# sangminwoo/Temporal-Span-Proposal-Network-VidVRD

Measured on AMD Instinct MI355X. Metric: tracklet-pairs/sec scored (N=32, T=150, D=2048), higher is better.
Workload: dtype f32

## Files before the change

### temporal-span-proposal-network-vidvrd_amd/csrc/tspn_wino63.hip

```cpp
#include <algorithm>
#include <atomic>
#include <type_traits>

#include "tspn_common.h"
#include "tspn_device.h"

namespace {

using namespace tspn_dev;

constexpr int NW = 4;
constexpr int THREADS = 64 * NW;
constexpr int BM = 128;
constexpr int ST = 32;
constexpr int SWG = 64;
constexpr int KC = 8;
constexpr int NJ = 8;
constexpr int VROW = ST * 4;
constexpr int VCH = 2 * NJ * VROW;
constexpr int VHALF = 4 * VCH;
constexpr int VSS = 2 * VHALF;
constexpr int NVB = 2;
constexpr int NPIECE = 16;
constexpr size_t SMEM_BYTES = sizeof(float) * NVB * VSS;
#ifndef TSPN_WINO63_GM
#define TSPN_WINO63_GM 4
#endif

#ifndef TSPN_WINO63_VAUX
#define TSPN_WINO63_VAUX 0
#endif

__global__ void pack_wino63_frag_kernel(const float* __restrict__ W, int64_t M, int64_t Cin, int64_t split,
                                        float* __restrict__ out) {
  const int64_t Mp = split ? 2 * M : M, Cp = split ? split : Cin;
  const int64_t nch = Cp / KC;
  const int64_t total = NJ * Cp * Mp;
  for (int64_t o = blockIdx.x * (int64_t)blockDim.x + threadIdx.x; o < total;
       o += (int64_t)gridDim.x * blockDim.x) {
    const int e = (int)(o & 3);
    const int lane = (int)((o >> 2) & 63);
    const int64_t r = o >> 8;
    const int j = (int)(r % NJ);
    const int64_t c = (r / NJ) % nch;
    const int64_t mb = r / (NJ * nch);
    const int64_t ch = 8 * c + 4 * (lane >> 5) + e;
    const int64_t m = 32 * mb + (lane & 31);
    const float* g = (split && m >= M) ? W + ((m - M) * Cin + split + ch) * 3 : W + (m * Cin + ch) * 3;
    const double g0 = g[0], g1 = g[1], g2 = g[2];
    double u;
    switch (j) {
      case 0: u = g0; break;
      case 1: u = -2.0 / 9.0 * (g0 + g1 + g2); break;
      case 2: u = -2.0 / 9.0 * (g0 - g1 + g2); break;
      case 3: u = g0 / 90.0 + g1 / 45.0 + 2.0 * g2 / 45.0; break;
      case 4: u = g0 / 90.0 - g1 / 45.0 + 2.0 * g2 / 45.0; break;
      case 5: u = (32.0 * g0 + 16.0 * g1 + 8.0 * g2) / 45.0; break;
      case 6: u = (32.0 * g0 - 16.0 * g1 + 8.0 * g2) / 45.0; break;
      default: u = g2; break;
    }
    out[o] = (float)u;
  }
}

__device__ __forceinline__ void wino63_load_sextet(const float* __restrict__ x, int64_t b, int q, int T, int Cin,
                                                   int64_t ncols, bool ok, int channel_offset, f32x4 (&d)[8]) {
#pragma unroll
  for (int i = 0; i < 8; ++i) {
    const int t = 6 * q + i - 1;
    int64_t n = b * T + t;
    n = n < 0 ? 0 : (n < ncols ? n : ncols - 1);
    const f32x4 v = *reinterpret_cast<const f32x4*>(x + n * Cin + channel_offset);
    d[i] = (ok && t >= 0 && t < T) ? v : f32x4{0.f, 0.f, 0.f, 0.f};
  }
}
__device__ __forceinline__ void wino63_bt(const f32x4 (&d)[8], f32x4 (&V)[8]) {
  V[0] = d[0] - d[6] + 5.25f * (d[4] - d[2]);
  V[7] = d[7] - d[1] + 5.25f * (d[3] - d[5]);
  {
    const f32x4 t1 = d[2] + d[6] - 4.25f * d[4], t2 = d[1] + d[5] - 4.25f * d[3];
    V[1] = t1 + t2;
    V[2] = t1 - t2;
  }
  {
    const f32x4 t1 = d[6] + 0.25f * d[2] - 1.25f * d[4], t2 = 0.5f * d[1] - 2.5f * d[3] + 2.f * d[5];
    V[3] = t1 + t2;
    V[4] = t1 - t2;
  }
  {
    const f32x4 t1 = d[6] + 4.f * (d[2] - 1.25f * d[4]), t2 = 2.f * d[1] - 2.5f * d[3] + 0.5f * d[5];
    V[5] = t1 + t2;
    V[6] = t1 - t2;
  }
}
__device__ __forceinline__ void wino63_absmax_own_frames(const f32x4 (&d)[8], float& m) {
#pragma unroll
  for (int i = 1; i < 7; ++i)
    m = __builtin_elementwise_maximum(
        __builtin_elementwise_maximum(m, __builtin_elementwise_maximum(fabsf(d[i][0]), fabsf(d[i][1]))),
        __builtin_elementwise_maximum(fabsf(d[i][2]), fabsf(d[i][3])));
}
__device__ __forceinline__ void wino63_hot_publish(unsigned long long* __restrict__ hot, unsigned long long key, unsigned slot) {
  key = tspn::wave_max_u64(key);
  if ((threadIdx.x & 63) == 0)
    __hip_atomic_fetch_max(hot + 32 * (slot & (TSPN_CONV_CHECK_HOT_SLOTS - 1)), key, __ATOMIC_RELAXED,
                           __HIP_MEMORY_SCOPE_AGENT);
}

__global__ __launch_bounds__(256) void wino63_input_transform_kernel(
    const float* __restrict__ x, float* __restrict__ Vg, int T, int Cin, int nq, int64_t nsext, int64_t nsp,
    int64_t ncols, unsigned long long* __restrict__ hot) {
  const int lane = threadIdx.x & 63, wave = threadIdx.x >> 6;
  const int cgl = lane & 7, ql = lane >> 3;
  const int64_t S = ((int64_t)blockIdx.x * 4 + wave) * 8 + ql;
  const int cg = blockIdx.y * 8 + cgl;
  if (4 * cg >= Cin) return;
  const bool ok = S < nsext;
  const int64_t b = ok ? S / nq : 0;
  const int q = ok ? (int)(S - b * nq) : 0;
  f32x4 d[8], V[8];
  wino63_load_sextet(x, b, q, T, Cin, ncols, ok, 4 * cg, d);
  if (hot) {
    float m = 0.f;
    wino63_absmax_own_frames(d, m);
    wino63_hot_publish(hot, ((unsigned long long)__float_as_uint(m) << 32) | (unsigned)(S < nsext ? S : 0),
                       blockIdx.x * 4 + wave + 7 * blockIdx.y);
  }
  wino63_bt(d, V);
#pragma unroll
  for (int j = 0; j < 8; ++j)
    *reinterpret_cast<f32x4*>(Vg + (((int64_t)cg * NJ + j) * nsp + S) * 4) = V[j];
}

template <bool BUFV>
__global__ __launch_bounds__(THREADS) __attribute__((amdgpu_waves_per_eu(1, 1))) void conv3_wino63_kernel(
    const float* __restrict__ Vg, const float* __restrict__ Wf, const float* __restrict__ bias,
    float* __restrict__ y, int Cin, int T, int M, int nq, int64_t nsext, int64_t nsp, int tiles_m,
    int tiles_n, int relu, int ldy, int GM, int vec2) {
  extern __shared__ __attribute__((aligned(16))) char smem_raw[];
  float* Vs = reinterpret_cast<float*>(smem_raw);

  int tile_m, tile_n;
  grouped_tile(xcd_remap(blockIdx.x, gridDim.x), GM, tiles_m, tiles_n, tile_m, tile_n);
  const int m0 = tile_m * BM;
  const int64_t S0 = (int64_t)tile_n * SWG;

  const int tid = threadIdx.x;
  const int lane = tid & 63;
  const int wave = __builtin_amdgcn_readfirstlane(tid >> 6);
  const int li = lane & 31, kh = lane >> 5;
  const int nsuper = Cin >> 5;

  const char* abase;
  const unsigned aoff = lane * 16;
  {
    int mb = (m0 >> 5) + wave;
    mb = mb < (M >> 5) ? mb : 0;
    abase = reinterpret_cast<const char*>(Wf) + (int64_t)mb * (Cin / KC) * (NJ * 64 * 16);
  }

  const float* vsrc[BUFV ? 1 : NPIECE];
  unsigned voff[BUFV ? NPIECE : 1];
#pragma unroll
  for (int k = 0; k < NPIECE; ++k) {
    const int pp = NPIECE * wave + k;
    const int rr = 2 * (pp & 31) + kh;
    const int cl = rr >> 4, rem = rr & 15;
    const int g = rem >> 3, j = rem & 7;
    const int64_t e = (((int64_t)(2 * cl + g) * NJ + j) * nsp + S0 + ST * (pp >> 5) + li) * 4;
    if constexpr (BUFV) voff[k] = (unsigned)(e * 4); else vsrc[k] = Vg + e;
  }
  const int64_t super_step = (int64_t)8 * NJ * nsp * 4;
  const __amdgpu_buffer_rsrc_t rsrc_v = buffer_rsrc(Vg, (int)0xffffffffu);
  const unsigned super_bytes = (unsigned)(super_step * 4);
  auto stage_piece = [&](int S, int k) {
    if constexpr (BUFV) {
      const int soff = (int)((unsigned)S * super_bytes);
      bglds16(rsrc_v, voff[k], soff, Vs + (S & 1) * VSS + (NPIECE * wave + k) * 256);
    } else {
      glds16<TSPN_WINO63_VAUX>(vsrc[k], Vs + (S & 1) * VSS + (NPIECE * wave + k) * 256);
    }
    if constexpr (!BUFV) vsrc[k] += super_step;
  };

  f32x16 acc[2][NJ];
#pragma unroll
  for (int cb = 0; cb < 2; ++cb)
#pragma unroll
    for (int j = 0; j < NJ; ++j)
#pragma unroll
      for (int e = 0; e < 16; ++e) acc[cb][j][e] = 0.f;

  f32x4 a[2][NJ], v[2][NJ];
  const float* vlane = Vs + (kh * NJ * ST + li) * 4;
  auto load_v = [&](const float* vbuf, int cl, int j) {
    v[0][j] = *reinterpret_cast<const f32x4*>(vbuf + cl * VCH + j * VROW);
    v[1][j] = *reinterpret_cast<const f32x4*>(vbuf + VHALF + cl * VCH + j * VROW);
  };
  auto load_a_pair = [&](f32x4* ap, auto jp_tag, const char* base) {
    constexpr int JP = decltype(jp_tag)::value;
    if (JP == 0) { load_wfrag<0>(ap[0], aoff, base); load_wfrag<1024>(ap[1], aoff, base); }
    if (JP == 1) { load_wfrag<2048>(ap[2], aoff, base); load_wfrag<3072>(ap[3], aoff, base); }
    if (JP == 2) { load_wfrag<0>(ap[4], aoff, base + 4096); load_wfrag<1024>(ap[5], aoff, base + 4096); }
    if (JP == 3) { load_wfrag<2048>(ap[6], aoff, base + 4096); load_wfrag<3072>(ap[7], aoff, base + 4096); }
  };
  using P0 = std::integral_constant<int, 0>;
  using P1 = std::integral_constant<int, 1>;
  using P2 = std::integral_constant<int, 2>;
  using P3 = std::integral_constant<int, 3>;
  auto mfma_pair = [&](const f32x4* ap, int ja, int jb, int S1, int slot) {
#pragma unroll
    for (int e = 0; e < 4; ++e) {
      acc[0][ja] = __builtin_amdgcn_mfma_f32_32x32x2f32(ap[ja][e], v[0][ja][e], acc[0][ja], 0, 0, 0);
      acc[0][jb] = __builtin_amdgcn_mfma_f32_32x32x2f32(ap[jb][e], v[0][jb][e], acc[0][jb], 0, 0, 0);
      acc[1][ja] = __builtin_amdgcn_mfma_f32_32x32x2f32(ap[ja][e], v[1][ja][e], acc[1][ja], 0, 0, 0);
      if (S1 >= 0) {
        __builtin_amdgcn_sched_barrier(0);
        stage_piece(S1, 4 * slot + e);
        __builtin_amdgcn_sched_barrier(0);
      }
      acc[1][jb] = __builtin_amdgcn_mfma_f32_32x32x2f32(ap[jb][e], v[1][jb][e], acc[1][jb], 0, 0, 0);
    }
  };

#pragma unroll
  for (int k = 0; k < NPIECE; ++k) stage_piece(0, k);
  asm volatile("s_waitcnt vmcnt(0)" ::: "memory");
  __syncthreads();
#pragma unroll
  for (int j = 0; j < NJ; ++j) load_v(vlane, 0, j);
  load_a_pair(a[0], P0{}, abase); load_a_pair(a[0], P1{}, abase); load_a_pair(a[0], P2{}, abase); load_a_pair(a[0], P3{}, abase);
  abase += NJ * 1024;
  load_a_pair(a[1], P0{}, abase); load_a_pair(a[1], P1{}, abase); load_a_pair(a[1], P2{}, abase); load_a_pair(a[1], P3{}, abase);
  abase += NJ * 1024;
  __builtin_amdgcn_sched_barrier(0);

  auto chunk_body = [&](auto cl_tag, const float* vcur, const float* vnext, int S, auto has1_tag, auto has2_tag,
                        auto more_tag) {
    constexpr int CL = decltype(cl_tag)::value;
    constexpr bool HAS1 = decltype(has1_tag)::value;
    constexpr bool HAS2 = decltype(has2_tag)::value;
    constexpr bool MORE = decltype(more_tag)::value;
    constexpr int PAR = CL & 1;
    constexpr int N1 = (HAS1 ? 8 : 0) + ((MORE && CL == 1) ? NPIECE : 0);
    constexpr int N2 = (MORE && CL == 2) ? 6 : 2;
    constexpr int N0 = (HAS2 ? 2 : 0) + ((MORE && CL == 0) ? 4 : 0);
    const int S1 = (MORE && CL == 0) ? S + 1 : -1;
    const float* vn = CL == 3 ? vnext : vcur;
    constexpr int NCL = (CL + 1) & 3;
    f32x4* ap = a[PAR];
    wait_w<3 * N2 + N1>(ap[0], ap[1]);
    mfma_pair(ap, 0, 1, S1, 0);
    if (HAS2) load_a_pair(ap, P0{}, abase);
    if (HAS1) { load_v(vn, NCL, 0); load_v(vn, NCL, 1); }
    __builtin_amdgcn_sched_barrier(0);
    wait_w<2 * N2 + N1 + N0>(ap[2], ap[3]);
    mfma_pair(ap, 2, 3, S1, 1);
    if (HAS2) load_a_pair(ap, P1{}, abase);
    if (HAS1) { load_v(vn, NCL, 2); load_v(vn, NCL, 3); }
    __builtin_amdgcn_sched_barrier(0);
    wait_w<N2 + N1 + 2 * N0>(ap[4], ap[5]);
    mfma_pair(ap, 4, 5, S1, 2);
    if (HAS2) load_a_pair(ap, P2{}, abase);
    if (HAS1) { load_v(vn, NCL, 4); load_v(vn, NCL, 5); }
    __builtin_amdgcn_sched_barrier(0);
    wait_w<N1 + 3 * N0>(ap[6], ap[7]);
    mfma_pair(ap, 6, 7, S1, 3);
    if (HAS2) {
      load_a_pair(ap, P3{}, abase);
      abase += NJ * 1024;
    }
    if (HAS1) { load_v(vn, NCL, 6); load_v(vn, NCL, 7); }
    __builtin_amdgcn_sched_barrier(0);
    if (MORE && CL == 2) {
      asm volatile("s_waitcnt lgkmcnt(0)" ::: "memory");
      __builtin_amdgcn_s_barrier();
      __builtin_amdgcn_sched_barrier(0);
    }
  };
  {
    using TT = std::true_type;
    using FF = std::false_type;
    using C0 = std::integral_constant<int, 0>;
    using C1 = std::integral_constant<int, 1>;
    using C2 = std::integral_constant<int, 2>;
    using C3 = std::integral_constant<int, 3>;
    int S = 0;
    for (; S + 1 < nsuper; ++S) {
      const float* vcur = vlane + (S & 1) * VSS;
      const float* vnext = vlane + ((S + 1) & 1) * VSS;
      chunk_body(C0{}, vcur, vnext, S, TT{}, TT{}, TT{});
      chunk_body(C1{}, vcur, vnext, S, TT{}, TT{}, TT{});
      chunk_body(C2{}, vcur, vnext, S, TT{}, TT{}, TT{});
      chunk_body(C3{}, vcur, vnext, S, TT{}, TT{}, TT{});
    }
    const float* vcur = vlane + (S & 1) * VSS;
    chunk_body(C0{}, vcur, vcur, S, TT{}, TT{}, FF{});
    chunk_body(C1{}, vcur, vcur, S, TT{}, TT{}, FF{});
    chunk_body(C2{}, vcur, vcur, S, TT{}, FF{}, FF{});
    chunk_body(C3{}, vcur, vcur, S, FF{}, FF{}, FF{});
  }

#pragma unroll
  for (int cb = 0; cb < 2; ++cb) {
    const int64_t Sx = S0 + ST * cb + li;
    if (Sx < nsext) {
      const int64_t b = Sx / nq;
      const int q = (int)(Sx - b * nq);
      const int t = 6 * q;
      float* ycol = y + (b * M) * (int64_t)ldy + t;
#pragma unroll
      for (int e = 0; e < 16; ++e) {
        const int m = m0 + wave * 32 + (e & 3) + 8 * (e >> 2) + 4 * kh;
        if (m < M) {
          const float p12 = acc[cb][1][e] + acc[cb][2][e], m12 = acc[cb][1][e] - acc[cb][2][e];
          const float p34 = acc[cb][3][e] + acc[cb][4][e], m34 = acc[cb][3][e] - acc[cb][4][e];
          const float p56 = acc[cb][5][e] + acc[cb][6][e], m56 = acc[cb][5][e] - acc[cb][6][e];
          float o[6];
          o[0] = acc[cb][0][e] + p12 + p34 + p56;
          o[1] = m12 + 2.f * m34 + 0.5f * m56;
          o[2] = p12 + 4.f * p34 + 0.25f * p56;
          o[3] = m12 + 8.f * m34 + 0.125f * m56;
          o[4] = p12 + 16.f * p34 + 0.0625f * p56;
          o[5] = m12 + 32.f * m34 + 0.03125f * m56 + acc[cb][7][e];
          if (bias != nullptr) {
            const float bb = bias[m];
#pragma unroll
            for (int i = 0; i < 6; ++i) o[i] += bb;
          }
          if (relu) {
#pragma unroll
            for (int i = 0; i < 6; ++i) o[i] = tspn::relu_f32(o[i]);
          }
          float* dst = ycol + (int64_t)m * ldy;
          if (vec2) {
            *reinterpret_cast<f32x2*>(dst) = f32x2{o[0], o[1]};
            *reinterpret_cast<f32x2*>(dst + 2) = f32x2{o[2], o[3]};
            *reinterpret_cast<f32x2*>(dst + 4) = f32x2{o[4], o[5]};
          } else {
#pragma unroll
            for (int i = 0; i < 6; ++i)
              if (t + i < T) dst[i] = o[i];
          }
        }
      }
    }
  }
}

constexpr int F_BM = 256, F_BN = 256;
constexpr int F_THREADS = 512;
constexpr int F_ST = 4 * 2 * 256 * 16;
constexpr int F_NST = 4;
constexpr size_t F_SMEM = (size_t)F_NST * F_ST;
constexpr size_t F_SMEM_ALL = F_SMEM + 2 * 256 * sizeof(int);
static_assert(TSPN_WINO63_GM > 0 && TSPN_WINO63_GM < 256, "the contraction's GM argument carries the tail split and the piece form above bit 7");
constexpr size_t F_PARK_PER_TILE = (size_t)7 * F_THREADS * 128 * sizeof(float);

__device__ __forceinline__ int split_exponent(double mx) {
  if (!(mx > 0.0) || !(mx <= 1.7976931348623157e308)) return 0;
  int k;
  (void)frexp(mx, &k);
  return 15 - k;
}

__device__ __forceinline__ double wino63_u(int j, double g0, double g1, double g2) {
  switch (j) {
    case 0: return g0;
    case 1: return -2.0 / 9.0 * (g0 + g1 + g2);
    case 2: return -2.0 / 9.0 * (g0 - g1 + g2);
    case 3: return g0 / 90.0 + g1 / 45.0 + 2.0 * g2 / 45.0;
    case 4: return g0 / 90.0 - g1 / 45.0 + 2.0 * g2 / 45.0;
    case 5: return (32.0 * g0 + 16.0 * g1 + 8.0 * g2) / 45.0;
    case 6: return (32.0 * g0 - 16.0 * g1 + 8.0 * g2) / 45.0;
    default: return g2;
  }
}

__global__ void pack_wino63_frag_kernel(const float* __restrict__ W, int64_t M, int64_t Cin, int64_t split,
                                        int16_t* __restrict__ out) {
  const int64_t Mp = split ? 2 * M : M, Cp = split ? split : Cin;
  const int64_t ncg = Cp / 8;
  const int64_t o = blockIdx.x * (int64_t)blockDim.x + threadIdx.x;
  if (o >= NJ * Mp) return;
  const int j = (int)(o / Mp);
  const int64_t m = o - j * Mp;
  const float* g = (split && m >= M) ? W + ((m - M) * Cin + split) * 3 : W + (m * Cin) * 3;
  double mx = 0.0;
  for (int64_t c = 0; c < Cp; ++c) {
    const double u = fabs(wino63_u(j, g[3 * c], g[3 * c + 1], g[3 * c + 2]));
    mx = (u > mx || u != u) ? u : mx;
  }
  const int e = split_exponent(mx);
  int16_t* pj = out + (int64_t)j * (2 * ncg + 1) * Mp * 8;
  for (int64_t cg = 0; cg < ncg; ++cg) {
    f16x8 hi, lo;
#pragma unroll
    for (int i = 0; i < 8; ++i) {
      const int64_t c = 8 * cg + i;
      const double u = ldexp(wino63_u(j, g[3 * c], g[3 * c + 1], g[3 * c + 2]), e);
      const _Float16 h = (_Float16)(float)u;
      hi[i] = h;
      lo[i] = (_Float16)(float)(u - (double)(float)h);
    }
    *reinterpret_cast<f16x8*>(pj + (cg * Mp + m) * 8) = hi;
    *reinterpret_cast<f16x8*>(pj + ((ncg + cg) * Mp + m) * 8) = lo;
  }
  *reinterpret_cast<int4*>(pj + (2 * ncg * Mp + m) * 8) = int4{e, 0, 0, 0};
}

__global__ __launch_bounds__(256) void wino63_input_transform_kernel(
    const float* __restrict__ x, _Float16* __restrict__ Vh, int* __restrict__ Ve, int T, int Cin, int nq,
    int64_t nsext, int64_t nsp2, int64_t ncols, unsigned long long* __restrict__ hot) {
  __shared__ float red[4][8][NJ];
  const int tid = threadIdx.x, lane = tid & 63, wave = tid >> 6;
  const int s = tid & 7, cgs = tid >> 3;
  const int64_t S = (int64_t)blockIdx.x * 8 + s;
  const bool ok = S < nsext;
  const int64_t b = ok ? S / nq : 0;
  const int q = ok ? (int)(S - b * nq) : 0;
  const int ncg = Cin >> 3;
  auto transform = [&](int cg, f32x4 (&V)[2][8], bool want_max, float& xmax) {
#pragma unroll
    for (int h = 0; h < 2; ++h) {
      f32x4 d[8];
      wino63_load_sextet(x, b, q, T, Cin, ncols, ok, 8 * cg + 4 * h, d);
      if (want_max) wino63_absmax_own_frames(d, xmax);
      wino63_bt(d, V[h]);
    }
  };
  float cmax[NJ];
#pragma unroll
  for (int j = 0; j < NJ; ++j) cmax[j] = 0.f;
  float xm = 0.f;
  for (int cg = cgs; cg < ncg; cg += 32) {
    f32x4 V[2][8];
    transform(cg, V, hot != nullptr, xm);
#pragma unroll
    for (int j = 0; j < NJ; ++j)
#pragma unroll
      for (int h = 0; h < 2; ++h)
        cmax[j] = __builtin_elementwise_maximum(
            __builtin_elementwise_maximum(cmax[j], __builtin_elementwise_maximum(fabsf(V[h][j][0]), fabsf(V[h][j][1]))),
            __builtin_elementwise_maximum(fabsf(V[h][j][2]), fabsf(V[h][j][3])));
  }
  if (hot)
    wino63_hot_publish(hot, ((unsigned long long)__float_as_uint(xm) << 32) | (unsigned)(ok ? S : 0),
                       blockIdx.x * 4 + wave);
#pragma unroll
  for (int j = 0; j < NJ; ++j) {
    float m = cmax[j];
#pragma unroll
    for (int o = 8; o < 64; o <<= 1) m = __builtin_elementwise_maximum(m, __shfl_xor(m, o, 64));
    if (lane < 8) red[wave][lane][j] = m;
  }
  __syncthreads();
  int ecol[NJ];
#pragma unroll
  for (int j = 0; j < NJ; ++j) {
    const float m = __builtin_elementwise_maximum(__builtin_elementwise_maximum(red[0][s][j], red[1][s][j]),
                                                  __builtin_elementwise_maximum(red[2][s][j], red[3][s][j]));
    ecol[j] = split_exponent((double)m);
  }
  if (cgs == 0) {
#pragma unroll
    for (int j = 0; j < NJ; ++j) Ve[(int64_t)j * nsp2 + S] = ecol[j];
  }
  for (int cg = cgs; cg < ncg; cg += 32) {
    f32x4 V[2][8];
    transform(cg, V, false, xm);
#pragma unroll
    for (int j = 0; j < NJ; ++j) {
      f16x8 hi, lo;
#pragma unroll
      for (int i = 0; i < 8; ++i) {
        const float u = ldexpf(V[i >> 2][j][i & 3], ecol[j]);
        const _Float16 h = (_Float16)u;
        hi[i] = h;
        lo[i] = (_Float16)(u - (float)h);
      }
      _Float16* dst = Vh + (((int64_t)j * 2 * ncg + cg) * nsp2 + S) * 8;
      *reinterpret_cast<f16x8*>(dst) = hi;
      *reinterpret_cast<f16x8*>(dst + (int64_t)ncg * nsp2 * 8) = lo;
    }
  }
}

#ifndef TSPN_WINO63_F16X3_STAGGER
#define TSPN_WINO63_F16X3_STAGGER 1
#endif
template <int WN, bool BUF>
__device__ __forceinline__ void wino63_f16x3_tile(
    char* smem_raw, const _Float16* __restrict__ Vh, const int* __restrict__ Ve, const int16_t* __restrict__ Wp,
    const float* __restrict__ bias, float* __restrict__ y, float* __restrict__ park, int Cin, int T, int M, int nq,
    int64_t nsext, int64_t nsp2, int tile_m, int tile_n, int tiles_n, int sub, int relu, int ldy, int vec2) {
  constexpr int MI = WN;
  constexpr int BN = 64 * WN;
  constexpr int NP = 16 + 4 * WN;
  constexpr int PW = (NP + 7) / 8;
  constexpr bool EVEN = NP % 8 == 0;
  constexpr bool STAGGER = TSPN_WINO63_F16X3_STAGGER && WN == 4;
  const int m0 = tile_m * F_BM;
  const int64_t S0 = (int64_t)tile_n * F_BN + sub * BN;

  const int tid = threadIdx.x;
  const int lane = tid & 63;
  const int wave = __builtin_amdgcn_readfirstlane(tid >> 6);
  const int wm = wave / WN, wn = wave % WN;
  const int li = lane & 31, kh = lane >> 5;
  const int ncg = Cin >> 3, nk = Cin >> 4;
  const int G = NJ * nk;

  const int p0 = wave * NP / 8;
  const int npw = EVEN ? PW : (wave + 1) * NP / 8 - p0;
  const int16_t* src[PW];
  unsigned voff[PW];
  int ldst[PW];
#pragma unroll
  for (int i = 0; i < PW; ++i) {
    const int p = min(p0 + i, NP - 1);
    int64_t el;
    if (p < 16) {
      const int region = p >> 3, cgi = (p >> 2) & 1, r = 64 * (p & 3) + lane;
      el = (((int64_t)region * ncg + cgi) * M + m0 + r) * 8;
      src[i] = Wp + el;
      ldst[i] = p * 1024;
    } else {
      const int v = p - 16;
      const int region = v / (2 * WN), cgi = (v / WN) & 1, r = 64 * (v % WN) + lane;
      el = (((int64_t)region * ncg + cgi) * nsp2 + S0 + r) * 8;
      src[i] = reinterpret_cast<const int16_t*>(Vh) + el;
      ldst[i] = (2 + region) * 8192 + cgi * 4096 + (v % WN) * 1024;
    }
    voff[i] = (unsigned)(el * 2);
  }
  int ik = 0, ist = 0;
  const char* wbase = reinterpret_cast<const char*>(Wp);
  const char* vbase = reinterpret_cast<const char*>(Vh);
  auto issue = [&]() {
    char* dst = smem_raw + ist * F_ST;
#pragma unroll
    for (int i = 0; i < PW; ++i)
      if (EVEN || i < npw) {
        if (BUF) bglds16(buffer_rsrc_unbounded(p0 + i < 16 ? wbase : vbase), voff[i], 0, dst + ldst[i]);
        else glds16(src[i], dst + ldst[i]);
      }
    ist = (ist + 1) & 3;
    const bool wrap = ++ik == nk;
    if (wrap) ik = 0;
    const int64_t dw = (int64_t)M * (wrap ? 32 * nk + 48 : 32), dv = nsp2 * (wrap ? 32 * nk + 32 : 32);
    if (BUF) {
      wbase += dw;
      vbase += dv;
    } else {
#pragma unroll
      for (int i = 0; i < PW; ++i) src[i] = reinterpret_cast<const int16_t*>(reinterpret_cast<const char*>(src[i]) + (p0 + i < 16 ? dw : dv));
    }
  };
  auto wait_stages = [&](auto ahead_tag) {
    constexpr int AHEAD = decltype(ahead_tag)::value;
    if (EVEN || npw == PW) wait_vmcnt<AHEAD * PW>(); else wait_vmcnt<AHEAD * (PW - 1)>();
  };

  f32x16 acc[MI][2];
#pragma unroll
  for (int mi = 0; mi < MI; ++mi)
#pragma unroll
    for (int ni = 0; ni < 2; ++ni)
#pragma unroll
      for (int e = 0; e < 16; ++e) acc[mi][ni][e] = 0.f;

  float* my_park = park + (int64_t)(tile_m * tiles_n + tile_n) * (F_PARK_PER_TILE / sizeof(float)) +
                   (int64_t)sub * (8 * MI) * F_THREADS * 4 + tid * 4;
  int* etab = reinterpret_cast<int*>(smem_raw + F_SMEM);
  auto unscale = [&](int j) {
    if (tid < F_BM)
      etab[tid] = reinterpret_cast<const int*>(Wp + (int64_t)j * (2 * ncg + 1) * M * 8 + (int64_t)2 * ncg * M * 8)[(int64_t)(m0 + tid) * 4];
    else if (tid - F_BM < BN)
      etab[tid] = Ve[(int64_t)j * nsp2 + S0 + tid - F_BM];
    __syncthreads();
    int ec[2];
#pragma unroll
    for (int ni = 0; ni < 2; ++ni) ec[ni] = etab[F_BM + wn * 64 + ni * 32 + li];
#pragma unroll
    for (int mi = 0; mi < MI; ++mi)
#pragma unroll
      for (int e = 0; e < 16; ++e) {
        const int r = etab[wm * (32 * MI) + mi * 32 + (e & 3) + 8 * (e >> 2) + 4 * kh];
#pragma unroll
        for (int ni = 0; ni < 2; ++ni) acc[mi][ni][e] = ldexpf(acc[mi][ni][e], -(r + ec[ni]));
      }
  };

  f16x8 ah[MI], al[MI], bh[2][2], bl[2];
  const int a_off = (kh * 256 + wm * (32 * MI) + li) * 16, b_off = (kh * 256 + wn * 64 + li) * 16;
  auto read_hi = [&](int st, f16x8 (&bhn)[2]) {
    const char* s = smem_raw + st * F_ST;
#pragma unroll
    for (int mi = 0; mi < MI; ++mi) ah[mi] = *reinterpret_cast<const f16x8*>(s + a_off + mi * 512);
#pragma unroll
    for (int ni = 0; ni < 2; ++ni) bhn[ni] = *reinterpret_cast<const f16x8*>(s + 16384 + b_off + ni * 512);
  };
  auto read_lo = [&](int st) {
    const char* s = smem_raw + st * F_ST;
#pragma unroll
    for (int ni = 0; ni < 2; ++ni) bl[ni] = *reinterpret_cast<const f16x8*>(s + 24576 + b_off + ni * 512);
#pragma unroll
    for (int mi = 0; mi < MI; ++mi) al[mi] = *reinterpret_cast<const f16x8*>(s + 8192 + a_off + mi * 512);
  };
  auto group = [&](const f16x8 (&a)[MI], const f16x8 (&b)[2]) {
#pragma unroll
    for (int ni = 0; ni < 2; ++ni)
#pragma unroll
      for (int mi = 0; mi < MI; ++mi) acc[mi][ni] = __builtin_amdgcn_mfma_f32_32x32x16_f16(a[mi], b[ni], acc[mi][ni], 0, 0, 0);
  };
  auto point_end = [&](int j) {
    unscale(j);
    if (j < NJ - 1) {
#pragma unroll
      for (int mi = 0; mi < MI; ++mi)
#pragma unroll
        for (int ni = 0; ni < 2; ++ni)
#pragma unroll
          for (int eq = 0; eq < 4; ++eq) {
            const f32x4 v = {acc[mi][ni][4 * eq], acc[mi][ni][4 * eq + 1], acc[mi][ni][4 * eq + 2], acc[mi][ni][4 * eq + 3]};
            *reinterpret_cast<f32x4*>(my_park + ((int64_t)j * 32 + (mi * 2 + ni) * 4 + eq) * F_THREADS * 4) = v;
#pragma unroll
            for (int e = 0; e < 4; ++e) acc[mi][ni][4 * eq + e] = 0.f;
          }
    }
    __builtin_amdgcn_sched_barrier(0);
  };
  auto kstep = [&](int g, f16x8 (&bc)[2], f16x8 (&bn)[2], auto steady_tag) {
    constexpr bool STEADY = decltype(steady_tag)::value;
#define TSPN_MR(NM, NR)                                \
  __builtin_amdgcn_sched_group_barrier(0x008, NM, 0);  \
  __builtin_amdgcn_sched_group_barrier(0x100, NR, 0);
    group(ah, bc);
    read_lo(g & 3);
    if (WN == 4) { TSPN_MR(1, 1) TSPN_MR(1, 1) TSPN_MR(1, 1) TSPN_MR(1, 1) TSPN_MR(1, 1) TSPN_MR(1, 1) TSPN_MR(2, 0) }
    __builtin_amdgcn_sched_barrier(0);
    if (STEADY || g + 2 < G) wait_stages(std::integral_constant<int, 1>{});
    else wait_vmcnt<0>();
    __builtin_amdgcn_s_barrier();
    __builtin_amdgcn_sched_barrier(0);
    const bool more = STEADY || g + 3 < G;
    if (more && (!STAGGER || wm == 0)) issue();
    __builtin_amdgcn_sched_barrier(0);
    group(ah, bl);
    __builtin_amdgcn_sched_barrier(0);
    if (STAGGER && more && wm != 0) issue();
    __builtin_amdgcn_sched_barrier(0);
    group(al, bc);
    if (STEADY || g + 1 < G) read_hi((g + 1) & 3, bn);
    if (WN == 4 && STEADY) { TSPN_MR(2, 1) TSPN_MR(1, 1) TSPN_MR(1, 1) TSPN_MR(1, 1) TSPN_MR(1, 1) TSPN_MR(1, 1) TSPN_MR(1, 0) }
#undef TSPN_MR
    __builtin_amdgcn_sched_barrier(0);
  };

  issue();
  issue();
  issue();
  wait_stages(std::integral_constant<int, 2>{});
  __builtin_amdgcn_s_barrier();
  __builtin_amdgcn_sched_barrier(0);
  read_hi(0, bh[0]);
  int g = 0, kc = 0, jc = 0;
  auto pair = [&](auto steady_tag) {
    kstep(g, bh[0], bh[1], steady_tag);
    kstep(g + 1, bh[1], bh[0], steady_tag);
    g += 2;
    kc += 2;
    if (kc == nk) {
      point_end(jc);
      kc = 0;
      ++jc;
    }
  };
  while (g + 4 < G) pair(std::true_type{});
  while (g < G) pair(std::false_type{});

  wait_vmcnt<0>();
#pragma unroll
  for (int ni = 0; ni < 2; ++ni) {
    const int64_t Sx = S0 + wn * 64 + ni * 32 + li;
    const bool col_ok = Sx < nsext;
    const int64_t b = col_ok ? Sx / nq : 0;
    const int q = col_ok ? (int)(Sx - b * nq) : 0;
    const int t = 6 * q;
    float* ycol = y + (b * M) * (int64_t)ldy + t;
#pragma unroll
    for (int mi = 0; mi < MI; ++mi)
#pragma unroll
      for (int eq = 0; eq < 4; ++eq) {
        f32x4 P[NJ - 1];
#pragma unroll
        for (int j = 0; j < NJ - 1; ++j)
          P[j] = *reinterpret_cast<const f32x4*>(my_park + ((int64_t)j * 32 + (mi * 2 + ni) * 4 + eq) * F_THREADS * 4);
        if (!col_ok) continue;
#pragma unroll
        for (int e4 = 0; e4 < 4; ++e4) {
          const int e = 4 * eq + e4;
          const int m = m0 + wm * (32 * MI) + mi * 32 + (e & 3) + 8 * (e >> 2) + 4 * kh;
          const float p12 = P[1][e4] + P[2][e4], m12 = P[1][e4] - P[2][e4];
          const float p34 = P[3][e4] + P[4][e4], m34 = P[3][e4] - P[4][e4];
          const float p56 = P[5][e4] + P[6][e4], m56 = P[5][e4] - P[6][e4];
          float o[6];
          o[0] = P[0][e4] + p12 + p34 + p56;
          o[1] = m12 + 2.f * m34 + 0.5f * m56;
          o[2] = p12 + 4.f * p34 + 0.25f * p56;
          o[3] = m12 + 8.f * m34 + 0.125f * m56;
          o[4] = p12 + 16.f * p34 + 0.0625f * p56;
          o[5] = m12 + 32.f * m34 + 0.03125f * m56 + acc[mi][ni][e];
          if (bias != nullptr) {
            const float bb = bias[m];
#pragma unroll
            for (int i = 0; i < 6; ++i) o[i] += bb;
          }
          if (relu) {
#pragma unroll
            for (int i = 0; i < 6; ++i) o[i] = tspn::relu_f32(o[i]);
          }
          float* dst = ycol + (int64_t)m * ldy;
          if (vec2) {
            *reinterpret_cast<f32x2*>(dst) = f32x2{o[0], o[1]};
            *reinterpret_cast<f32x2*>(dst + 2) = f32x2{o[2], o[3]};
            *reinterpret_cast<f32x2*>(dst + 4) = f32x2{o[4], o[5]};
          } else {
#pragma unroll
            for (int i = 0; i < 6; ++i)
              if (t + i < T) dst[i] = o[i];
          }
        }
      }
  }
}

__global__ __launch_bounds__(F_THREADS, 1) void conv3_wino63_kernel(
    const _Float16* __restrict__ Vh, const int* __restrict__ Ve, const int16_t* __restrict__ Wp,
    const float* __restrict__ bias, float* __restrict__ y, float* __restrict__ park, int Cin, int T, int M, int nq,
    int64_t nsext, int64_t nsp2, int tiles_m, int tiles_n, int relu, int ldy, int GM, int vec2) {
  extern __shared__ __attribute__((aligned(16))) char smem_raw[];

  const int f = max((GM >> 8) & 0xff, 1);
  const bool buf = (GM >> 16) & 1;
  GM &= 0xff;
  const int tiles = tiles_m * tiles_n;
  const int nsplit = f > 1 ? ((int)gridDim.x - tiles) / (f - 1) : 0;
  const int nfull = tiles - nsplit;
  const int bid = blockIdx.x;
  int wg, sub = 0;
  if (bid < nfull) {
    wg = xcd_remap(bid, nfull);
  } else {
    const int s = xcd_remap(bid - nfull, nsplit * f);
    wg = nfull + s / f;
    sub = s - (s / f) * f;
  }
  int tile_m, tile_n;
  grouped_tile(wg, GM, tiles_m, tiles_n, tile_m, tile_n);
  auto tile = [&](auto wn_tag, auto buf_tag) {
    wino63_f16x3_tile<decltype(wn_tag)::value, decltype(buf_tag)::value>(
        smem_raw, Vh, Ve, Wp, bias, y, park, Cin, T, M, nq, nsext, nsp2, tile_m, tile_n, tiles_n, sub, relu, ldy, vec2);
  };
  auto shape = [&](auto buf_tag) {
    if (bid < nfull) tile(std::integral_constant<int, 4>{}, buf_tag);
    else if (f == 2) tile(std::integral_constant<int, 2>{}, buf_tag);
    else tile(std::integral_constant<int, 1>{}, buf_tag);
  };
  if (buf) shape(std::true_type{}); else shape(std::false_type{});
}

int64_t padded_sextets(int64_t B, int64_t T) { return tspn::ceil_div(B * tspn::ceil_div(T, 6), SWG) * SWG; }
int64_t padded_sextets_f16x3(int64_t B, int64_t T) { return tspn::ceil_div(B * tspn::ceil_div(T, 6), F_BN) * F_BN; }

struct F16x3Layout {
  size_t v, e, park, total;
};
F16x3Layout f16x3_layout(int64_t B, int64_t T, int64_t Cin, int64_t M) {
  F16x3Layout L{};
  const size_t nsp2 = (size_t)padded_sextets_f16x3(B, T);
  L.v = 0;
  L.e = tspn::align_up((size_t)NJ * 2 * Cin * nsp2 * sizeof(_Float16), 256);
  L.park = L.e + tspn::align_up((size_t)NJ * nsp2 * sizeof(int), 256);
  L.total = L.park + (size_t)tspn::ceil_div(M, F_BM) * (nsp2 / F_BN) * F_PARK_PER_TILE;
  return L;
}

int check_common(const char* what, int64_t B, int64_t T, int64_t Cin, int64_t M, int64_t ldy) {
  TSPN_REQUIRE(B >= 0 && Cin > 0 && T > 0 && M > 0 && ldy >= T && ldy < (1 << 24), TSPN_EINVAL,
               "%s: bad sizes B=%lld T=%lld Cin=%lld M=%lld ldy=%lld", what, (long long)B, (long long)T,
               (long long)Cin, (long long)M, (long long)ldy);
  TSPN_REQUIRE(tspn::wino63_supported(Cin, M), TSPN_EUNSUPPORTED,
               "%s: needs Cin %% 32 == 0, M %% 32 == 0 (Cin=%lld M=%lld)", what, (long long)Cin, (long long)M);
  TSPN_REQUIRE(Cin < (1 << 24) && T < (1 << 24) && M < (1 << 24), TSPN_EUNSUPPORTED, "%s: dimension too large", what);
  return TSPN_OK;
}

}

bool tspn::wino63_supported(int64_t Cin, int64_t M) { return Cin > 0 && M > 0 && Cin % 32 == 0 && M % 32 == 0; }

size_t tspn::wino63_workspace_bytes(int64_t B, int64_t T, int64_t Cin) {
  if (B <= 0 || T <= 0 || Cin <= 0 || Cin % 32 != 0) return 0;
  return (size_t)(Cin / 4) * NJ * (size_t)padded_sextets(B, T) * 4 * sizeof(float);
}

extern "C" size_t tspn_conv3_tc_wino63_workspace_bytes(int64_t B, int64_t T, int64_t Cin) {
  return tspn::wino63_workspace_bytes(B, T, Cin);
}

extern "C" int tspn_pack_conv3_wino63_frag_f32(const float* W, int64_t M, int64_t Cin, int64_t split, float* frag,
                                               void* stream) {
  TSPN_REQUIRE(W && frag, TSPN_EINVAL, "tspn_pack_conv3_wino63_frag_f32: null pointer");
  TSPN_REQUIRE(M > 0 && Cin > 0 && split >= 0, TSPN_EINVAL, "tspn_pack_conv3_wino63_frag_f32: bad sizes");
  TSPN_REQUIRE(split == 0 || Cin == 2 * split, TSPN_EINVAL,
               "tspn_pack_conv3_wino63_frag_f32: split=%lld requires Cin == 2*split (Cin=%lld)", (long long)split,
               (long long)Cin);
  const int64_t Mp = split ? 2 * M : M, Cp = split ? split : Cin;
  TSPN_REQUIRE(Cp % KC == 0 && Mp % 32 == 0, TSPN_EUNSUPPORTED,
               "tspn_pack_conv3_wino63_frag_f32: needs (packed) Cin %% 8 == 0 and M %% 32 == 0 (Cin=%lld M=%lld)",
               (long long)Cp, (long long)Mp);
  const int64_t total = NJ * Cp * Mp;
  const int blocks = (int)std::min<int64_t>(tspn::ceil_div(total, 256), 8192);
  hipLaunchKernelGGL(pack_wino63_frag_kernel, dim3(blocks), dim3(256), 0, TSPN_STREAM(stream), W, M, Cin, split, frag);
  return tspn::check_launch("tspn_pack_conv3_wino63_frag_f32");
}

int tspn::wino63_input_transform(const float* x, int64_t B, int64_t T, int64_t Cin, void* workspace,
                                 size_t workspace_bytes, void* stream, uint64_t* hot) {
  const char* what = "tspn_conv3_tc_wino63_f32(input transform)";
  if (int rc = check_common(what, B, T, Cin, 32, T)) return rc;
  if (B == 0) return TSPN_OK;
  TSPN_REQUIRE(x && tspn::aligned16(x), TSPN_EINVAL, "%s: x must be a 16-byte aligned pointer", what);
  const size_t need = tspn::wino63_workspace_bytes(B, T, Cin);
  TSPN_REQUIRE(workspace && workspace_bytes >= need, TSPN_EWORKSPACE, "%s: workspace %zu < %zu bytes", what,
               workspace_bytes, need);
  TSPN_REQUIRE(tspn::aligned16(workspace), TSPN_EINVAL, "%s: workspace must be 16-byte aligned",
               what);
  const int64_t nq = tspn::ceil_div(T, 6);
  const int64_t nsext = B * nq, nsp = padded_sextets(B, T);
  TSPN_REQUIRE(nsp / 32 < (1LL << 31) && Cin / 32 < 65536, TSPN_EUNSUPPORTED, "%s: grid too large", what);
  hipLaunchKernelGGL(wino63_input_transform_kernel, dim3((unsigned)(nsp / 32), (unsigned)(Cin / 32)), dim3(256), 0,
                     TSPN_STREAM(stream), x, static_cast<float*>(workspace), (int)T, (int)Cin, (int)nq, nsext, nsp,
                     B * T, reinterpret_cast<unsigned long long*>(hot));
  return tspn::check_launch(what);
}

static std::atomic<int> g_piece_form{0};

int tspn::wino63_contract(const void* workspace, int64_t B, int64_t T, int64_t Cin, const float* frag, int64_t M,
                          const float* bias, int relu, float* y, int64_t ldy, void* stream) {
  const char* what = "tspn_conv3_tc_wino63_f32";
  if (int rc = check_common(what, B, T, Cin, M, ldy)) return rc;
  if (B == 0) return TSPN_OK;
  TSPN_REQUIRE(workspace && frag && y, TSPN_EINVAL, "%s: null pointer", what);
  TSPN_REQUIRE(tspn::aligned16(frag) && (reinterpret_cast<uintptr_t>(y) & 3) == 0,
               TSPN_EUNSUPPORTED, "%s: frag must be 16-byte aligned", what);
  const int64_t nq = tspn::ceil_div(T, 6);
  const int64_t nsext = B * nq, nsp = padded_sextets(B, T);
  const int64_t tiles_m = tspn::ceil_div(M, BM), tiles_n = nsp / SWG;
  TSPN_REQUIRE(tiles_m * tiles_n < (1LL << 31), TSPN_EUNSUPPORTED, "%s: grid too large", what);
  const int vec2 = (ldy % 2 == 0) && (ldy >= 6 * nq) && ((reinterpret_cast<uintptr_t>(y) & 7) == 0);
#ifndef TSPN_WINO63_BUFV
#define TSPN_WINO63_BUFV 1
#endif
  const bool bufv = TSPN_WINO63_BUFV && tspn::wino63_workspace_bytes(B, T, Cin) < (1ull << 32) &&
                    g_piece_form.load(std::memory_order_relaxed) == 0;
  static tspn::LdsLimit lds[2];
  auto launch = [&](auto kern, tspn::LdsLimit& lim) {
    if (int rc = lim.ensure(reinterpret_cast<const void*>(kern), SMEM_BYTES, what)) return rc;
    hipLaunchKernelGGL(kern, dim3((unsigned)(tiles_m * tiles_n)), dim3(THREADS), SMEM_BYTES, TSPN_STREAM(stream),
                       static_cast<const float*>(workspace), frag, bias, y, (int)Cin, (int)T, (int)M, (int)nq, nsext, nsp,
                       (int)tiles_m, (int)tiles_n, relu, (int)ldy, TSPN_WINO63_GM, vec2);
    return tspn::check_launch(what);
  };
  return bufv ? launch(conv3_wino63_kernel<true>, lds[1]) : launch(conv3_wino63_kernel<false>, lds[0]);
}

int tspn::conv3_tc_wino63(const float* x, int64_t B, int64_t T, int64_t Cin, const float* frag, int64_t M,
                          const float* bias, int relu, float* y, int64_t ldy, void* workspace,
                          size_t workspace_bytes, void* stream) {
  if (int rc = check_common("tspn_conv3_tc_wino63_f32", B, T, Cin, M, ldy)) return rc;
  if (int rc = tspn::wino63_input_transform(x, B, T, Cin, workspace, workspace_bytes, stream)) return rc;
  return tspn::wino63_contract(workspace, B, T, Cin, frag, M, bias, relu, y, ldy, stream);
}

extern "C" int tspn_conv3_tc_wino63_set_piece_form(int form) {
  TSPN_REQUIRE(form == 0 || form == 1, TSPN_EINVAL, "tspn_conv3_tc_wino63_set_piece_form: form must be 0 or 1");
  return g_piece_form.exchange(form, std::memory_order_relaxed);
}

extern "C" int tspn_conv3_tc_wino63_f32(const float* x, int64_t B, int64_t T, int64_t Cin, const float* frag,
                                        int64_t M, const float* bias, int relu, float* y, void* workspace,
                                        size_t workspace_bytes, void* stream) {
  return tspn::conv3_tc_wino63(x, B, T, Cin, frag, M, bias, relu, y, T, workspace, workspace_bytes, stream);
}

bool tspn::wino63_f16x3_supported(int64_t Cin, int64_t M) {
  return Cin > 0 && M > 0 && Cin % 32 == 0 && M % F_BM == 0 && Cin < (1 << 24) && M < (1 << 24);
}

size_t tspn::wino63_f16x3_workspace_bytes(int64_t B, int64_t T, int64_t Cin, int64_t M) {
  if (B <= 0 || T <= 0 || !tspn::wino63_f16x3_supported(Cin, M)) return 0;
  return f16x3_layout(B, T, Cin, M).total;
}

extern "C" size_t tspn_conv3_tc_wino63_f16x3_workspace_bytes(int64_t B, int64_t T, int64_t Cin, int64_t M) {
  return tspn::wino63_f16x3_workspace_bytes(B, T, Cin, M);
}

extern "C" size_t tspn_pack_conv3_wino63_f16x3_elements(int64_t M, int64_t Cin, int64_t split) {
  if (M <= 0 || Cin <= 0 || split < 0 || (split && Cin != 2 * split)) return 0;
  const int64_t Mp = split ? 2 * M : M, Cp = split ? split : Cin;
  return (size_t)NJ * (2 * (Cp / 8) + 1) * Mp * 8;
}

extern "C" int tspn_pack_conv3_wino63_f16x3(const float* W, int64_t M, int64_t Cin, int64_t split, int16_t* packed,
                                            void* stream) {
  const char* what = "tspn_pack_conv3_wino63_f16x3";
  TSPN_REQUIRE(W && packed, TSPN_EINVAL, "%s: null pointer", what);
  TSPN_REQUIRE(M > 0 && Cin > 0 && split >= 0, TSPN_EINVAL, "%s: bad sizes", what);
  TSPN_REQUIRE(split == 0 || Cin == 2 * split, TSPN_EINVAL, "%s: split=%lld requires Cin == 2*split (Cin=%lld)", what,
               (long long)split, (long long)Cin);
  TSPN_REQUIRE(tspn::aligned16(packed), TSPN_EINVAL, "%s: packed must be 16-byte aligned", what);
  const int64_t Mp = split ? 2 * M : M, Cp = split ? split : Cin;
  TSPN_REQUIRE(tspn::wino63_f16x3_supported(Cp, Mp), TSPN_EUNSUPPORTED,
               "%s: needs (packed) Cin %% 32 == 0 and M %% 256 == 0 (Cin=%lld M=%lld)", what, (long long)Cp, (long long)Mp);
  void (*kern)(const float*, int64_t, int64_t, int64_t, int16_t*) = pack_wino63_frag_kernel;
  hipLaunchKernelGGL(kern, dim3((unsigned)tspn::ceil_div(NJ * Mp, 256)), dim3(256), 0, TSPN_STREAM(stream), W, M, Cin,
                     split, packed);
  return tspn::check_launch(what);
}

int tspn::wino63_f16x3_input_transform(const float* x, int64_t B, int64_t T, int64_t Cin, int64_t M, void* workspace,
                                       size_t workspace_bytes, void* stream, uint64_t* hot) {
  const char* what = "tspn_conv3_tc_wino63_f16x3(input transform)";
  if (int rc = check_common(what, B, T, Cin, 32, T)) return rc;
  TSPN_REQUIRE(tspn::wino63_f16x3_supported(Cin, M), TSPN_EUNSUPPORTED,
               "%s: needs Cin %% 32 == 0 and M %% 256 == 0 (Cin=%lld M=%lld)", what, (long long)Cin, (long long)M);
  if (B == 0) return TSPN_OK;
  TSPN_REQUIRE(x && tspn::aligned16(x), TSPN_EINVAL, "%s: x must be a 16-byte aligned pointer", what);
  const F16x3Layout L = f16x3_layout(B, T, Cin, M);
  TSPN_REQUIRE(workspace && workspace_bytes >= L.total, TSPN_EWORKSPACE, "%s: workspace %zu < %zu bytes", what,
               workspace_bytes, L.total);
  TSPN_REQUIRE((reinterpret_cast<uintptr_t>(workspace) & 255) == 0, TSPN_EINVAL, "%s: workspace must be 256-byte aligned",
               what);
  const int64_t nq = tspn::ceil_div(T, 6);
  const int64_t nsext = B * nq, nsp2 = padded_sextets_f16x3(B, T);
  TSPN_REQUIRE(nsp2 / 8 < (1LL << 31), TSPN_EUNSUPPORTED, "%s: grid too large", what);
  char* ws = static_cast<char*>(workspace);
  void (*kern)(const float*, _Float16*, int*, int, int, int, int64_t, int64_t, int64_t, unsigned long long*) =
      wino63_input_transform_kernel;
  hipLaunchKernelGGL(kern, dim3((unsigned)(nsp2 / 8)), dim3(256), 0, TSPN_STREAM(stream), x,
                     reinterpret_cast<_Float16*>(ws + L.v), reinterpret_cast<int*>(ws + L.e), (int)T, (int)Cin, (int)nq,
                     nsext, nsp2, B * T, reinterpret_cast<unsigned long long*>(hot));
  return tspn::check_launch(what);
}

static std::atomic<int> g_tail_split{1};

extern "C" int tspn_conv3_tc_wino63_f16x3_set_tail_split(int on) {
  TSPN_REQUIRE(on == 0 || on == 1, TSPN_EINVAL, "tspn_conv3_tc_wino63_f16x3_set_tail_split: on must be 0 or 1");
  return g_tail_split.exchange(on, std::memory_order_relaxed);
}

static int device_cus() {
  constexpr int kMaxDevices = 64;
  static std::atomic<int> cached[kMaxDevices] = {};
  int dev = -1, cus = 0;
  if (hipGetDevice(&dev) != hipSuccess) return 0;
  const bool tracked = dev >= 0 && dev < kMaxDevices;
  if (tracked && (cus = cached[dev].load(std::memory_order_relaxed)) > 0) return cus;
  if (hipDeviceGetAttribute(&cus, hipDeviceAttributeMultiprocessorCount, dev) != hipSuccess || cus <= 0) return 0;
  if (tracked) cached[dev].store(cus, std::memory_order_relaxed);
  return cus;
}

static int tail_split_factor(int64_t tiles, int cus, int64_t* R) {
  *R = 0;
  if (cus <= 0 || g_tail_split.load(std::memory_order_relaxed) == 0) return 1;
  const int64_t r = tiles % cus;
  if (r == 0) return 1;
  const int64_t f = std::min<int64_t>(4, cus / r);
  if (f < 2) return 1;
  *R = r;
  return f == 3 ? 2 : (int)f;
}

int tspn::wino63_f16x3_contract(void* workspace, size_t workspace_bytes, int64_t B, int64_t T, int64_t Cin,
                                const int16_t* packed, int64_t M, const float* bias, int relu, float* y, int64_t ldy,
                                void* stream) {
  const char* what = "tspn_conv3_tc_wino63_f16x3";
  if (int rc = check_common(what, B, T, Cin, M, ldy)) return rc;
  TSPN_REQUIRE(tspn::wino63_f16x3_supported(Cin, M), TSPN_EUNSUPPORTED,
               "%s: needs Cin %% 32 == 0 and M %% 256 == 0 (Cin=%lld M=%lld)", what, (long long)Cin, (long long)M);
  if (B == 0) return TSPN_OK;
  TSPN_REQUIRE(workspace && packed && y, TSPN_EINVAL, "%s: null pointer", what);
  TSPN_REQUIRE(tspn::aligned16(packed) && (reinterpret_cast<uintptr_t>(y) & 3) == 0,
               TSPN_EUNSUPPORTED, "%s: packed weights must be 16-byte aligned", what);
  const F16x3Layout L = f16x3_layout(B, T, Cin, M);
  TSPN_REQUIRE(workspace_bytes >= L.total, TSPN_EWORKSPACE, "%s: workspace %zu < %zu bytes", what, workspace_bytes,
               L.total);
  const int64_t nq = tspn::ceil_div(T, 6);
  const int64_t nsext = B * nq, nsp2 = padded_sextets_f16x3(B, T);
  const int64_t tiles_m = M / F_BM, tiles_n = nsp2 / F_BN;
  TSPN_REQUIRE(tiles_m * tiles_n < (1LL << 29), TSPN_EUNSUPPORTED, "%s: grid too large", what);
  const int vec2 = (ldy % 2 == 0) && (ldy >= 6 * nq) && ((reinterpret_cast<uintptr_t>(y) & 7) == 0);
  int64_t R = 0;
  const int f = tail_split_factor(tiles_m * tiles_n, device_cus(), &R);
  const int64_t grid = tiles_m * tiles_n + R * (f - 1);
  const int64_t slab = 4 * Cin * std::max<int64_t>(M, nsp2);
  const int buf = slab < (1LL << 31) && g_piece_form.load(std::memory_order_relaxed) == 0;
  char* ws = static_cast<char*>(workspace);
  static tspn::LdsLimit lds;
  void (*kern)(const _Float16*, const int*, const int16_t*, const float*, float*, float*, int, int, int, int, int64_t,
               int64_t, int, int, int, int, int, int) = conv3_wino63_kernel;
  if (int rc = lds.ensure(reinterpret_cast<const void*>(kern), F_SMEM_ALL, what)) return rc;
  hipLaunchKernelGGL(kern, dim3((unsigned)grid), dim3(F_THREADS), F_SMEM_ALL, TSPN_STREAM(stream),
                     reinterpret_cast<const _Float16*>(ws + L.v), reinterpret_cast<const int*>(ws + L.e), packed, bias, y,
                     reinterpret_cast<float*>(ws + L.park), (int)Cin, (int)T, (int)M, (int)nq, nsext, nsp2, (int)tiles_m,
                     (int)tiles_n, relu, (int)ldy, TSPN_WINO63_GM | (f << 8) | (buf << 16), vec2);
  return tspn::check_launch(what);
}

extern "C" int tspn_conv3_tc_wino63_f16x3(const float* x, int64_t B, int64_t T, int64_t Cin, const int16_t* packed,
                                          int64_t M, const float* bias, int relu, float* y, void* workspace,
                                          size_t workspace_bytes, void* stream) {
  const char* what = "tspn_conv3_tc_wino63_f16x3";
  if (int rc = check_common(what, B, T, Cin, M, T)) return rc;
  TSPN_REQUIRE(tspn::wino63_f16x3_supported(Cin, M), TSPN_EUNSUPPORTED,
               "%s: needs Cin %% 32 == 0 and M %% 256 == 0 (Cin=%lld M=%lld)", what, (long long)Cin, (long long)M);
  if (B > 0) {
    TSPN_REQUIRE(workspace && packed && y, TSPN_EINVAL, "%s: null pointer", what);
    TSPN_REQUIRE(tspn::aligned16(packed) && (reinterpret_cast<uintptr_t>(y) & 3) == 0,
                 TSPN_EUNSUPPORTED, "%s: packed weights must be 16-byte aligned", what);
  }
  if (int rc = tspn::wino63_f16x3_input_transform(x, B, T, Cin, M, workspace, workspace_bytes, stream)) return rc;
  return tspn::wino63_f16x3_contract(workspace, workspace_bytes, B, T, Cin, packed, M, bias, relu, y, T, stream);
}
```

Baseline: 1.222 million.

## Defer Winograd point unscaling to epilogue, removing per-point block barriers

Per-point exponent unscaling, which needed a global load, a __syncthreads and ldexp over all accumulators after each of the eight Winograd points, moves into the final epilogue. There, exponent tables for all points and the bias are staged once into the reused pipeline shared memory. Parked partial sums are stored unscaled and rescaled as they are read back. This removes eight block-wide barriers from the main MFMA loop and shrinks the dynamic LDS request, at the cost of a heavier epilogue with more LDS reads.

```diff
diff --git a/temporal-span-proposal-network-vidvrd_amd/csrc/tspn_wino63.hip b/temporal-span-proposal-network-vidvrd_amd/csrc/tspn_wino63.hip
--- a/temporal-span-proposal-network-vidvrd_amd/csrc/tspn_wino63.hip
+++ b/temporal-span-proposal-network-vidvrd_amd/csrc/tspn_wino63.hip
@@ -353,7 +353,6 @@
 constexpr int F_ST = 4 * 2 * 256 * 16;
 constexpr int F_NST = 4;
 constexpr size_t F_SMEM = (size_t)F_NST * F_ST;
-constexpr size_t F_SMEM_ALL = F_SMEM + 2 * 256 * sizeof(int);
 static_assert(TSPN_WINO63_GM > 0 && TSPN_WINO63_GM < 256, "the contraction's GM argument carries the tail split and the piece form above bit 7");
 constexpr size_t F_PARK_PER_TILE = (size_t)7 * F_THREADS * 128 * sizeof(float);
 
@@ -572,26 +571,6 @@
 
   float* my_park = park + (int64_t)(tile_m * tiles_n + tile_n) * (F_PARK_PER_TILE / sizeof(float)) +
                    (int64_t)sub * (8 * MI) * F_THREADS * 4 + tid * 4;
-  int* etab = reinterpret_cast<int*>(smem_raw + F_SMEM);
-  auto unscale = [&](int j) {
-    if (tid < F_BM)
-      etab[tid] = reinterpret_cast<const int*>(Wp + (int64_t)j * (2 * ncg + 1) * M * 8 + (int64_t)2 * ncg * M * 8)[(int64_t)(m0 + tid) * 4];
-    else if (tid - F_BM < BN)
-      etab[tid] = Ve[(int64_t)j * nsp2 + S0 + tid - F_BM];
-    __syncthreads();
-    int ec[2];
-#pragma unroll
-    for (int ni = 0; ni < 2; ++ni) ec[ni] = etab[F_BM + wn * 64 + ni * 32 + li];
-#pragma unroll
-    for (int mi = 0; mi < MI; ++mi)
-#pragma unroll
-      for (int e = 0; e < 16; ++e) {
-        const int r = etab[wm * (32 * MI) + mi * 32 + (e & 3) + 8 * (e >> 2) + 4 * kh];
-#pragma unroll
-        for (int ni = 0; ni < 2; ++ni) acc[mi][ni][e] = ldexpf(acc[mi][ni][e], -(r + ec[ni]));
-      }
-  };
-
   f16x8 ah[MI], al[MI], bh[2][2], bl[2];
   const int a_off = (kh * 256 + wm * (32 * MI) + li) * 16, b_off = (kh * 256 + wn * 64 + li) * 16;
   auto read_hi = [&](int st, f16x8 (&bhn)[2]) {
@@ -615,7 +594,6 @@
       for (int mi = 0; mi < MI; ++mi) acc[mi][ni] = __builtin_amdgcn_mfma_f32_32x32x16_f16(a[mi], b[ni], acc[mi][ni], 0, 0, 0);
   };
   auto point_end = [&](int j) {
-    unscale(j);
     if (j < NJ - 1) {
 #pragma unroll
       for (int mi = 0; mi < MI; ++mi)
@@ -681,14 +659,30 @@
   while (g < G) pair(std::false_type{});
 
   wait_vmcnt<0>();
-#pragma unroll
-  for (int ni = 0; ni < 2; ++ni) {
-    const int64_t Sx = S0 + wn * 64 + ni * 32 + li;
+  __syncthreads();
+  constexpr int ET = F_BM + BN;
+  int* etab = reinterpret_cast<int*>(smem_raw);
+#pragma unroll
+  for (int j = 0; j < NJ; ++j) {
+    if (tid < F_BM)
+      etab[j * ET + tid] = reinterpret_cast<const int*>(Wp + (int64_t)j * (2 * ncg + 1) * M * 8 + (int64_t)2 * ncg * M * 8)[(int64_t)(m0 + tid) * 4];
+    else if (tid - F_BM < BN)
+      etab[j * ET + tid] = Ve[(int64_t)j * nsp2 + S0 + tid - F_BM];
+  }
+  float* btab = reinterpret_cast<float*>(etab + NJ * ET);
+  if (bias != nullptr && tid < F_BM) btab[tid] = bias[m0 + tid];
+  __syncthreads();
+  auto read_back = [&](auto ni_tag) {
+    constexpr int NI = decltype(ni_tag)::value;
+    const int64_t Sx = S0 + wn * 64 + NI * 32 + li;
     const bool col_ok = Sx < nsext;
     const int64_t b = col_ok ? Sx / nq : 0;
     const int q = col_ok ? (int)(Sx - b * nq) : 0;
     const int t = 6 * q;
     float* ycol = y + (b * M) * (int64_t)ldy + t;
+    int ec[NJ];
+#pragma unroll
+    for (int j = 0; j < NJ; ++j) ec[j] = etab[j * ET + F_BM + wn * 64 + NI * 32 + li];
 #pragma unroll
     for (int mi = 0; mi < MI; ++mi)
 #pragma unroll
@@ -696,24 +690,31 @@
         f32x4 P[NJ - 1];
 #pragma unroll
         for (int j = 0; j < NJ - 1; ++j)
-          P[j] = *reinterpret_cast<const f32x4*>(my_park + ((int64_t)j * 32 + (mi * 2 + ni) * 4 + eq) * F_THREADS * 4);
+          P[j] = *reinterpret_cast<const f32x4*>(my_park + ((int64_t)j * 32 + (mi * 2 + NI) * 4 + eq) * F_THREADS * 4);
         if (!col_ok) continue;
+        const int* er = etab + wm * (32 * MI) + mi * 32 + 8 * eq + 4 * kh;
+        f32x4 bb4 = {0.f, 0.f, 0.f, 0.f};
+        if (bias != nullptr) bb4 = *reinterpret_cast<const f32x4*>(btab + wm * (32 * MI) + mi * 32 + 8 * eq + 4 * kh);
 #pragma unroll
         for (int e4 = 0; e4 < 4; ++e4) {
           const int e = 4 * eq + e4;
           const int m = m0 + wm * (32 * MI) + mi * 32 + (e & 3) + 8 * (e >> 2) + 4 * kh;
-          const float p12 = P[1][e4] + P[2][e4], m12 = P[1][e4] - P[2][e4];
-          const float p34 = P[3][e4] + P[4][e4], m34 = P[3][e4] - P[4][e4];
-          const float p56 = P[5][e4] + P[6][e4], m56 = P[5][e4] - P[6][e4];
+          float Mj[NJ];
+#pragma unroll
+          for (int j = 0; j < NJ - 1; ++j) Mj[j] = ldexpf(P[j][e4], -(er[j * ET + e4] + ec[j]));
+          Mj[7] = ldexpf(acc[mi][NI][e], -(er[7 * ET + e4] + ec[7]));
+          const float p12 = Mj[1] + Mj[2], m12 = Mj[1] - Mj[2];
+          const float p34 = Mj[3] + Mj[4], m34 = Mj[3] - Mj[4];
+          const float p56 = Mj[5] + Mj[6], m56 = Mj[5] - Mj[6];
           float o[6];
-          o[0] = P[0][e4] + p12 + p34 + p56;
+          o[0] = Mj[0] + p12 + p34 + p56;
           o[1] = m12 + 2.f * m34 + 0.5f * m56;
           o[2] = p12 + 4.f * p34 + 0.25f * p56;
           o[3] = m12 + 8.f * m34 + 0.125f * m56;
           o[4] = p12 + 16.f * p34 + 0.0625f * p56;
-          o[5] = m12 + 32.f * m34 + 0.03125f * m56 + acc[mi][ni][e];
+          o[5] = m12 + 32.f * m34 + 0.03125f * m56 + Mj[7];
           if (bias != nullptr) {
-            const float bb = bias[m];
+            const float bb = bb4[e4];
 #pragma unroll
             for (int i = 0; i < 6; ++i) o[i] += bb;
           }
@@ -733,7 +734,9 @@
           }
         }
       }
-  }
+  };
+  read_back(std::integral_constant<int, 0>{});
+  read_back(std::integral_constant<int, 1>{});
 }
 
 __global__ __launch_bounds__(F_THREADS, 1) void conv3_wino63_kernel(
@@ -1016,8 +1019,8 @@
   static tspn::LdsLimit lds;
   void (*kern)(const _Float16*, const int*, const int16_t*, const float*, float*, float*, int, int, int, int, int64_t,
                int64_t, int, int, int, int, int, int) = conv3_wino63_kernel;
-  if (int rc = lds.ensure(reinterpret_cast<const void*>(kern), F_SMEM_ALL, what)) return rc;
-  hipLaunchKernelGGL(kern, dim3((unsigned)grid), dim3(F_THREADS), F_SMEM_ALL, TSPN_STREAM(stream),
+  if (int rc = lds.ensure(reinterpret_cast<const void*>(kern), F_SMEM, what)) return rc;
+  hipLaunchKernelGGL(kern, dim3((unsigned)grid), dim3(F_THREADS), F_SMEM, TSPN_STREAM(stream),
                      reinterpret_cast<const _Float16*>(ws + L.v), reinterpret_cast<const int*>(ws + L.e), packed, bias, y,
                      reinterpret_cast<float*>(ws + L.park), (int)Cin, (int)T, (int)M, (int)nq, nsext, nsp2, (int)tiles_m,
                      (int)tiles_n, relu, (int)ldy, TSPN_WINO63_GM | (f << 8) | (buf << 16), vec2);
```

Result: no change. 1.211 million (-0.9%).
